# gafniguy/4D-Facial-Avatars

Hardware: AMD Instinct MI355X
Metric: rays/sec at 512x512, 64 coarse + 128 fine samples (higher is better)
Workload: dtype f32; 1 GPU; configs[1]: paper-model eval forward, 512x512 frame, 64+128 samples, chunksize 65536, perturb on, expression+latent conditioned, background prior; frames sharded over GPUs

## Files before the change

4d-facial-avatars_amd/csrc/nf_mlp_gated_stats.hip:

```cpp
#include "nf_mlp_live_kernel.h"

extern "C" int nf_paper_mlp_fwd_gated_stats(const float* packed, const float* bound, const float* cond, const float* ro, const float* rd,
                                            const float* rd_view, const float* z, int64_t n_rays, int n_samples, float* raw, float* scratch,
                                            size_t scratch_floats, int max_workgroups, int64_t* stats, size_t stats_rows, nf_stream_t stream) {
    static_assert(sizeof(long long) == sizeof(int64_t), "a statistics row is five int64");
    if (max_workgroups < 0 || !stats || ((uintptr_t)stats & 7) || stats_rows < (size_t)nf_live_grid_cap(max_workgroups) * NF_MLP_WAVES) return NF_EINVAL;
    const hipError_t e = hipMemsetAsync(stats, 0, stats_rows * NF_GATE_STAT_COLS * sizeof(int64_t), nf_s(stream));
    if (e != hipSuccess) return (int)e;
    return nf_live_launch<true, true>(packed, cond, ro, rd, rd_view, z, n_rays, n_samples, raw, scratch, scratch_floats, max_workgroups,
                                      reinterpret_cast<long long*>(stats), stream, bound);
}
```

4d-facial-avatars_amd/csrc/nf_mlp_live_kernel.h:

```cpp
#pragma once
#include <mutex>
#include "nf_mlp_paper_net.h"

#define NF_LIVE_ROWS 64
#ifndef NF_LIVE_PF
#define NF_LIVE_PF 8
#endif
#define NF_LIVE_DIR_B (NF_LIVE_ROWS * 1024)
#define NF_LIVE_META_B (NF_LIVE_DIR_B + NF_LIVE_ROWS * 64)
#define NF_LIVE_WAVE_B (NF_LIVE_META_B + NF_LIVE_ROWS * 16)
#define NF_LIVE_OOB NF_LIVE_WAVE_B
#define NF_LIVE_SC1 16

static_assert(NF_LIVE_ROWS == 64 && NF_MLP_NT == 2, "row numbers wrap with & 63; a pass's liveness is one 32-bit mask");
static_assert(NF_LIVE_PF >= 0 && NF_LIVE_PF <= 16, "prefetched rows live in registers beside fc_alpha's weights");

__device__ __forceinline__ __amdgpu_buffer_rsrc_t nf_live_ring(char* ring_v) {
    const uint64_t a = (uint64_t)ring_v;
    const uint64_t s = (uint64_t)(uint32_t)__builtin_amdgcn_readfirstlane((int)(uint32_t)a) |
                       ((uint64_t)(uint32_t)__builtin_amdgcn_readfirstlane((int)(a >> 32)) << 32);
    return __builtin_amdgcn_make_buffer_rsrc(reinterpret_cast<char*>(s), (short)0, NF_LIVE_WAVE_B, 0x00020000);
}
__device__ __forceinline__ void nf_live_store(__amdgpu_buffer_rsrc_t ring, int off_b, f32x4 v) {
    __builtin_amdgcn_raw_buffer_store_b128(__builtin_bit_cast(nf_u32x4, v), ring, off_b, 0, 0);
// ... 55 lines not shown
        const __amdgpu_buffer_rsrc_t ring = nf_live_ring(ring_v);
        const int tail = __builtin_amdgcn_readfirstlane(tail_v), cnt = __builtin_amdgcn_readfirstlane(head_v) - tail;
#pragma unroll
        for (int i = 0; i < NF_LIVE_PF; ++i)
            pf[i] = nf_live_load(ring, i < cnt ? ((tail + i) & (NF_LIVE_ROWS - 1)) * 1024 + lane * 16 : NF_LIVE_OOB);
        nf_load_bias<16>(st.bias, Ci, Net::B_FEAT, lane);
        nf_load_w16<16>(st.wa, Wi, Net::OFF_FEAT / 4, lane);
        __builtin_amdgcn_sched_barrier(0);
    }
};

#define NF_LIVE_STAT_UNITS 0
#define NF_LIVE_STAT_RUNS 1
#define NF_LIVE_STAT_FLUSH 2
#define NF_LIVE_STAT_CLOCK 3
#define NF_LIVE_STAT_COLS 4
#define NF_GATE_STAT_PROVEN 4
#define NF_GATE_STAT_COLS 5

template <bool STATS, int COLS = NF_LIVE_STAT_COLS>
__device__ __forceinline__ void nf_live_stat(long long* stats, int col, long long add, bool set = false) {
    if constexpr (STATS) {
        if ((threadIdx.x & 63) == 0) {
            long long* at = stats + ((size_t)blockIdx.x * NF_MLP_WAVES + (threadIdx.x >> 6)) * COLS + col;
            *at = set ? add : *at + add;
        }
    }
}

template <int NT, bool STATS, bool GATE = false>
__global__ void __launch_bounds__(64 * NF_MLP_WAVES, 1)
k_paper_mlp_fwd_live(const float* __restrict__ packed, const float* __restrict__ cond_, const float* __restrict__ ro,
                     const float* __restrict__ rd, const float* __restrict__ rd_view, const float* __restrict__ z,
                     int64_t n_points, int S, float* __restrict__ raw, float* __restrict__ scratch, unsigned* __restrict__ counter,
                     long long* __restrict__ stats, const float* __restrict__ bound) {
    using Net = NfPaperNet;
    constexpr int COLS = GATE ? NF_GATE_STAT_COLS : NF_LIVE_STAT_COLS;
    __shared__ __attribute__((aligned(16))) f32x4 lds[NF_MLP_WAVES * 16 * NT * 64];
    const int lane = threadIdx.x & 63, wave = threadIdx.x >> 6;
    f32x4* act4 = lds + wave * (16 * NT * 64);
    typedef __attribute__((address_space(1))) f32x4 nf_gf32x4;
    nf_gf32x4* raw_v = (nf_gf32x4*)raw;
    asm volatile("" : "+v"(raw_v));
// ... 22 lines not shown
        const bool more = __builtin_amdgcn_readfirstlane(more_v) != 0;
        unsigned next_v = 0;
        if (more && lane == 0) next_v = __hip_atomic_fetch_add(ctr_v, 1u, __ATOMIC_RELAXED, __HIP_MEMORY_SCOPE_AGENT);
        if (more) nf_live_stat<STATS, COLS>(stats, NF_LIVE_STAT_UNITS, 1);
        int opaque0 = 0;
        asm volatile("" : "+s"(opaque0));
        const NfW Wi = nf_w_image(packed + opaque0, Net::PACKED), Ci = nf_w_image(cond_ + opaque0, Net::COND_FLOATS);
        NfStream<NT> st;
        f32x4 wd[16], pf[NF_LIVE_PF > 0 ? NF_LIVE_PF : 1];
        f32x4 dirf[NT][1];
        float sigma_own[NT];
        float tag_own[NT] = {};
        bool proven[NT] = {};
        int live_v = 0, run_v = 0;
        if (more) {
            f32x4 pe[NT][4];
            nf_net_inputs<NT>(pe, dirf, p0, n_points, S, lane, ro, rd, rdv_v, z_v);
            f32x4 acc[NT][16];
            if constexpr (GATE) {
                nf_paper_net_body<Net, NT, 1, true, NfGatePre, true>(acc, sigma_own, pe, dirf, Wi, Ci, act4, lane,
                                                                     NfGatePre{st, pf, ring_v, head_v, tail_v, bound_v});
#pragma unroll
                for (int t = 0; t < NT; ++t) {
                    const float s = acc[t][8].x, u = acc[t][8].y;
                    sigma_own[t] = nf_add(s, nf_mul(u, 0x1p-13f));
                    proven[t] = sigma_own[t] < -0x1p-100f && s > -INFINITY && u < INFINITY;
                }
            } else {
                nf_paper_net_body<Net, NT, 1, true>(acc, sigma_own, pe, dirf, Wi, Ci, act4, lane, NfLivePre{st, wd, pf, ring_v, head_v, tail_v});
            }
            int lane_o = lane;
            asm volatile("" : "+v"(lane_o));
            const int g = lane_o >> 4, c = lane_o & 15;
            unsigned live = 0;
            int S_o = S;
            asm volatile("" : "+v"(S_o));
            const int64_t p0_o = (int64_t)(uint32_t)__builtin_amdgcn_readfirstlane((int)(uint32_t)p0_v) |
                                 ((int64_t)__builtin_amdgcn_readfirstlane((int)(p0_v >> 32)) << 32);
#pragma unroll
            for (int t = 0; t < NT; ++t) {
                const int64_t p = p0_o + 16 * t + c;
                const bool is_live = g == 0 && p < n_points && ((GATE ? !proven[t] : !(sigma_own[t] <= 0.0f)) || (p + 1) % S_o == 0);
                if constexpr (GATE) tag_own[t] = __int_as_float((p + 1) % S_o == 0 ? 1 : 0);
                live |= ((unsigned)__builtin_amdgcn_ballot_w64(is_live) & 0xffffu) << (16 * t);
            }
            const int head = __builtin_amdgcn_readfirstlane(head_v), cnt = head - __builtin_amdgcn_readfirstlane(tail_v);
            const int n_live = __builtin_popcount(live);
            live_v = (int)live;
            if constexpr (GATE) {
                const int64_t left = n_points - p0_o;
                nf_live_stat<STATS, COLS>(stats, NF_GATE_STAT_PROVEN, (left < 16 * NT ? (int)left : 16 * NT) - n_live);
            }
            if (cnt + n_live >= 16 * NT) {
                run_v = 1;
            } else {
                const __amdgpu_buffer_rsrc_t ring = nf_live_ring(ring_v);
                unsigned mm = live;
#pragma unroll 1
// ... 14 lines not shown
                for (int t = 0; t < NT; ++t) {
                    const int bit = 16 * t + c;
                    if ((live >> bit) & 1u) {
                        const int row = (head + __builtin_popcount(live & ((1u << bit) - 1u))) & (NF_LIVE_ROWS - 1);
                        nf_live_store(ring, NF_LIVE_DIR_B + row * 64 + g * 16, dirf[t][0]);
                        if (g == 0) {
                            const int64_t p = p0_o + bit;
                            nf_live_store(ring, NF_LIVE_META_B + row * 16,
                                          (f32x4){__int_as_float((int)(uint32_t)p), __int_as_float((int)(p >> 32)), GATE ? tag_own[t] : sigma_own[t], 0.0f});
                        }
                    }
                }
                head_v = head + n_live;
                asm volatile("" : "+v"(head_v));
            }
        } else {
            if constexpr (GATE) {
                NfGatePre pre{st, pf, ring_v, head_v, tail_v, bound_v};
                pre.wait();
                pre.loads(Wi, Ci, lane);
            } else {
                NfLivePre pre{st, wd, pf, ring_v, head_v, tail_v};
                pre.wait();
                pre.loads(Wi, Ci, lane);
            }
#pragma unroll
            for (int t = 0; t < NT; ++t) {
                dirf[t][0] = (f32x4){0.0f, 0.0f, 0.0f, 0.0f};
                sigma_own[t] = 0.0f;
            }
            run_v = __builtin_amdgcn_readfirstlane(head_v) != __builtin_amdgcn_readfirstlane(tail_v) ? 2 : 0;
        }
        asm volatile("" : "+v"(live_v), "+v"(run_v));
        const int run = __builtin_amdgcn_readfirstlane(run_v);
        if (run != 0) {
            nf_live_stat<STATS, COLS>(stats, NF_LIVE_STAT_RUNS, 1);
            if (run == 2) nf_live_stat<STATS, COLS>(stats, NF_LIVE_STAT_FLUSH, __builtin_amdgcn_readfirstlane(head_v) - __builtin_amdgcn_readfirstlane(tail_v));
            int lane_o = lane;
            asm volatile("" : "+v"(lane_o));
            const int g = lane_o >> 4, c = lane_o & 15;
            const __amdgpu_buffer_rsrc_t ring = nf_live_ring(ring_v);
            const int tail = __builtin_amdgcn_readfirstlane(tail_v), cnt = __builtin_amdgcn_readfirstlane(head_v) - tail;
            const unsigned own = run == 1 ? (unsigned)__builtin_amdgcn_readfirstlane(live_v) : 0u;
            const unsigned fill = run == 1 ? ~own : (1u << cnt) - 1u;
            const int n_fill = __builtin_popcount(fill);
            f32x4 meta[NT];
            bool valid[NT];
#pragma unroll
            for (int t = 0; t < NT; ++t) {
                const int bit = 16 * t + c;
                const bool f = (fill >> bit) & 1u;
                const int row = (tail + __builtin_popcount(fill & ((1u << bit) - 1u))) & (NF_LIVE_ROWS - 1);
// ... 17 lines not shown
                f32x4 v[4];
                int h[4];
#pragma unroll
                for (int u = 0; u < 4; ++u) {
                    const bool ok = i + u < n_fill;
                    h[u] = ok ? nf_live_pop(hh) : -1;
                    v[u] = nf_live_load(ring, ok ? ((tail + i + u) & (NF_LIVE_ROWS - 1)) * 1024 + lane_o * 16 : NF_LIVE_OOB);
                }
#pragma unroll
                for (int u = 0; u < 4; ++u)
                    if (h[u] >= 0) act4[nf_live_slab(h[u], lane_o)] = v[u];
            }
            constexpr int NDIR = 1;
            constexpr unsigned D0 = Net::OFF_D0 / 4;
            nf_read_b<NT>(st.b0, act4, lane, 0);
            f32x4 acc[NT][16], bj[NT];
            float sigma_raw[NT];
            if constexpr (GATE) {
                nf_seg_lds<NT, 16, true, true>(acc, st, Wi, Net::OFF_FEAT / 4, 16, act4, lane);
                nf_pending_b<NT, true>(bj, st);
                nf_tail<NT, 16, 16, 9, 1>(acc, st.wb, bj, st, Wi, D0, Ci, Net::B_D0, act4, lane);
                NF_NET_COLOUR();
            } else {
                NF_NET_COLOUR_D0(8, 9, wd);
                NF_NET_COLOUR_REST();
            }
            int lane_s = lane;
            asm volatile("" : "+v"(lane_s));
            if ((lane_s >> 4) == 0) {
#pragma unroll
                for (int t = 0; t < NT; ++t) {
                    if (valid[t]) {
                        const int64_t p = (int64_t)(uint32_t)__float_as_int(meta[t].x) | ((int64_t)__float_as_int(meta[t].y) << 32);
                        if constexpr (GATE) {
                            const bool keep = !(sigma_raw[t] <= 0.0f) || __float_as_int(meta[t].z) != 0;
                            if (p >= 0 && p < n_points)
                                raw_v[p] = (f32x4){keep ? acc[t][0].x : 0.0f, keep ? acc[t][0].y : 0.0f, keep ? acc[t][0].z : 0.0f, sigma_raw[t]};
                        } else {
                            if (p >= 0 && p < n_points) raw_v[p] = (f32x4){acc[t][0].x, acc[t][0].y, acc[t][0].z, meta[t].z};
                        }
                    }
                }
            }
            tail_v = tail + n_fill;
            asm volatile("" : "+v"(tail_v));
        }
        asm volatile("" : "+v"(more_v));
        if (__builtin_amdgcn_readfirstlane(more_v) == 0) break;
        {
            int lane_s = lane;
            asm volatile("" : "+v"(lane_s));
            const int g = lane_s >> 4, c = lane_s & 15;
            asm volatile("" : "+v"(live_v));
#pragma unroll
            for (int t = 0; t < NT; ++t) {
                const int64_t p = p0_v + 16 * t + c;
                if (g == 0 && p < n_points && !(((unsigned)live_v >> (16 * t + c)) & 1u)) raw_v[p] = (f32x4){0.0f, 0.0f, 0.0f, sigma_own[t]};
            }
        }
        asm volatile("" : "+v"(next_v));
        unit_v = next_v;
    }
    nf_live_stat<STATS, COLS>(stats, NF_LIVE_STAT_CLOCK, (long long)wall_clock64(), true);
}

static inline int64_t nf_live_grid_cap(int max_workgroups) {
    const int64_t cu = nf_cu_count();
    return max_workgroups > 0 && max_workgroups < cu ? max_workgroups : cu;
}

#define NF_LIVE_SLOTS 256
#define NF_LIVE_SLOT_B 128

// ... 23 lines not shown
    int i = 0;
    while (i < p.used && p.owner[i] != key) ++i;
    if (i == p.used) {
        if (p.used == NF_LIVE_SLOTS) {
            if (hipDeviceSynchronize() != hipSuccess) return nullptr;
            p.used = i = 0;
        }
        p.owner[p.used++] = key;
    }
    return reinterpret_cast<unsigned*>(p.base + (size_t)i * NF_LIVE_SLOT_B);
}

template <bool STATS, bool GATE = false>
static inline int nf_live_launch(const float* packed, const float* cond, const float* ro, const float* rd, const float* rd_view, const float* z,
                                 int64_t n_rays, int n_samples, float* raw, float* scratch, size_t scratch_floats, int max_workgroups,
                                 long long* stats, nf_stream_t stream, const float* bound = nullptr) {
    static_assert(NF_MLP_WAVES * 16 * NF_MLP_NT == 128, "nf_mlp_fwd_launch sizes the grid for 128 points per workgroup");
    if (max_workgroups < 0 || !scratch || ((uintptr_t)scratch & 15) ||
        scratch_floats < (size_t)nf_live_grid_cap(max_workgroups) * NF_MLP_WAVES * (NF_LIVE_WAVE_B / 4) ||
        (GATE && (!bound || ((uintptr_t)bound & 15))))
        return NF_EINVAL;
    const float* rdv = rd_view ? rd_view : rd;
    int rc = 0;
    const int launched = nf_mlp_fwd_launch(NF_FWD_INFER, packed, cond, ro, rd, z, raw, nullptr, n_rays, n_samples, [&](int64_t n_points, unsigned grid) {
        if ((n_points + 31) / 32 > ((int64_t)1 << 31)) {
            rc = NF_EINVAL;
            return;
        }
        unsigned* counter = nf_live_counter(nf_s(stream));
        if (!counter) {
            rc = (int)hipErrorOutOfMemory;
            return;
        }
        const hipError_t e = hipMemsetAsync(counter, 0, sizeof(unsigned), nf_s(stream));
        if (e != hipSuccess) {
            rc = (int)e;
            return;
// ... 8 lines not shown
```

4d-facial-avatars_amd/csrc/nf_mlp_live_stats.hip:

```cpp
#include "nf_mlp_live_kernel.h"

extern "C" int nf_paper_mlp_fwd_live_stats(const float* packed, const float* cond, const float* ro, const float* rd, const float* rd_view,
                                           const float* z, int64_t n_rays, int n_samples, float* raw, float* scratch, size_t scratch_floats,
                                           int max_workgroups, int64_t* stats, size_t stats_rows, nf_stream_t stream) {
    static_assert(sizeof(long long) == sizeof(int64_t), "a statistics row is four int64");
    if (max_workgroups < 0 || !stats || ((uintptr_t)stats & 7) || stats_rows < (size_t)nf_live_grid_cap(max_workgroups) * NF_MLP_WAVES) return NF_EINVAL;
    const hipError_t e = hipMemsetAsync(stats, 0, stats_rows * NF_LIVE_STAT_COLS * sizeof(int64_t), nf_s(stream));
    if (e != hipSuccess) return (int)e;
    return nf_live_launch<true>(packed, cond, ro, rd, rd_view, z, n_rays, n_samples, raw, scratch, scratch_floats, max_workgroups,
                                reinterpret_cast<long long*>(stats), stream);
}
```

4d-facial-avatars_amd/csrc/nf_mlp_paper_net.h:

```cpp
#pragma once
#include "nf_mlp_net_common.h"
#include "nf_mlp_smaller_layout.h"
#include "nf_pack.h"

#define NF_NET_COMMON(F)                                                                                                              \
    F(FRAG) F(NCOND) F(OFF_L0) F(OFF_L1) F(OFF_L2) F(OFF_L3) F(OFF_L4) F(OFF_FEAT) F(OFF_D0) F(OFF_D0E) F(OFF_D1) F(OFF_D2) F(OFF_RGB) \
    F(OFF_WC0) F(OFF_WC3) F(OFF_WCD) F(OFF_BIAS) F(B_L0) F(B_L1) F(B_L2) F(B_L3) F(B_L4) F(B_FEAT) F(B_D0) F(B_D1) F(B_D2) F(B_RGB)     \
    F(B_CVEC) F(B_DVEC) F(COND_FLOATS) F(S_PE) F(S_H0) F(S_H1) F(S_H2) F(S_H3) F(S_H4) F(S_FEAT) F(S_D0) F(S_D1) F(S_D2) F(S_DIRF)     \
    F(S_MASK) F(SAVED_PER_POINT) F(Z_L0) F(Z_L1) F(Z_L2) F(Z_L3) F(Z_L4) F(Z_FEAT) F(Z_D0) F(Z_D1) F(Z_D2) F(DZ_PER_POINT)             \
    F(OFFT_RGB) F(OFFT_D2) F(OFFT_D1) F(OFFT_D0) F(OFFT_FEAT) F(OFFT_L4) F(OFFT_L3) F(OFFT_L2) F(OFFT_L1)                              \
    F(G_L0) F(G_L1) F(G_L2) F(G_L3A) F(G_L3B) F(G_L4) F(G_FEAT) F(G_D0A) F(G_D0B) F(G_D1) F(G_D2) F(G_RGB) F(G_ALPHA)                  \
    F(CS_L0) F(CS_D0) F(CS_RGB) F(SLAB_FLOATS) F(GRAD_PARAM_FLOATS) F(GRAD_FLOATS)

struct NfPaperNet {
#define NF_NET_COPY(X) static constexpr int X = nfl::X;
    NF_NET_COMMON(NF_NET_COPY)
    NF_NET_COPY(OFF_L5) NF_NET_COPY(B_L5) NF_NET_COPY(S_H5) NF_NET_COPY(Z_L5) NF_NET_COPY(OFFT_L5) NF_NET_COPY(G_L5)
#undef NF_NET_COPY
    static constexpr bool HAS_L5 = true, D0_EXPR = false;
    static constexpr int PACKED = nfl::PACKED_FLOATS, PACKED_T = nfl::PACKED_T_FLOATS, NPARAMS = NF_PAPER_NUM_PARAMS;
    static constexpr int N_RELU = (nfl::SAVED_PER_POINT - nfl::S_MASK) / 8;
    static constexpr int D0_COLS = 280;
    static constexpr int MODEL = 0;
};
// ... 181 lines not shown

struct NfNoPre {
    __device__ __forceinline__ void wait() const {}
    __device__ __forceinline__ void loads(const NfW&, const NfW&, int) const {}
};
#define NF_BOUND_BIAS 4096
#define NF_BOUND_FLOATS (NF_BOUND_BIAS + 16)
template <int NT, bool RELU_IN, class Pre>
__device__ __forceinline__ void nf_net_lone_tile(f32x4 (&acc)[NT][16], const NfStream<NT>& st, f32x4 (&bj)[NT], const NfW& W, unsigned first4,
                                                 unsigned stride4, const NfW& Wi, const NfW& Ci, const f32x4* act4, int lane, Pre& pre) {
    f32x4 w8[16];
    w8[0] = st.wa[0];
    pre.wait();
#pragma unroll
    for (int ch = 1; ch < 16; ++ch) w8[ch] = nf_load_w1(W, first4 + stride4 * ch, lane);
    pre.loads(Wi, Ci, lane);
#pragma unroll
    for (int ch = 0; ch < 16; ++ch) {
        if (ch == 0) {
#pragma unroll
            for (int t = 0; t < NT; ++t) bj[t] = RELU_IN ? nf_relu_i(st.b0[t]) : st.b0[t];
        } else {
            nf_read_b<NT>(bj, act4, lane, ch);
            if (RELU_IN) {
#pragma unroll
                for (int t = 0; t < NT; ++t) bj[t] = nf_relu_i(bj[t]);
            }
        }
#pragma unroll
        for (int r = 0; r < 4; ++r)
#pragma unroll
// ... 236 lines not shown
```

4d-facial-avatars_amd/nerf/_hip.py:

```python
from __future__ import annotations

import ctypes as C
import os
import threading

import torch

_LIB_PATH = os.environ.get("NERFACE_HIP_LIB") or os.path.join(os.path.dirname(os.path.dirname(os.path.abspath(__file__))), "lib",
                                                             "libnerface_hip.so")
_lib = None
_lock = threading.Lock()

NF_PAPER_NUM_PARAMS = 26

_P, _I, _L, _F, _Z = C.c_void_p, C.c_int, C.c_int64, C.c_float, C.c_size_t
_PROTOTYPES = {
    "nf_abi_version": (C.c_int, []),
    "nf_error_string": (C.c_char_p, [_I]),
    "nf_build_info": (C.c_char_p, []),
    "nf_ray_bundle": (C.c_int, [_I, _I, _F, _F, _F, _F, _P, _I, _P, _P, _P]),
    "nf_weighted_choice_workspace_bytes": (_Z, []),
    "nf_weighted_choice": (C.c_int, [_P, _P, _L, _I, _P, _P, _Z, _P]),
    "nf_ray_batch": (C.c_int, [_I, _I, _F, _F, _F, _F, _P, _I, _P, _I, _L, _P, _I, _P, _P, _P, _P, _P, _P, _P]),
    "nf_sample_coarse": (C.c_int, [_L, _I, _F, _F, _P, _P, _P, _P]),
# ... 151 lines not shown
    "forward_encoded": (C.c_int, [_P, _P, _P, _P, _L, _P, _P, _P]),
}
for _prefix in ("nf_bshape", "nf_cbshape"):
    _PROTOTYPES.update({f"{_prefix}_{_name}": _sig for _name, _sig in _FAMILY_ENTRY_POINTS.items()})
_SIGMA_SIG = (C.c_int, [_P, _P, _P, _P, _P, _P, _L, _I, _P, _P])
SIGMA_ENTRY_POINTS = tuple(f"{_prefix}_mlp_sigma{_suffix}" for _prefix in ("nf_paper", "nf_lcode", "nf_bshape", "nf_cbshape")
                           for _suffix in ("", "_bf16", "_f16", "_f16x2")) + ("nf_smaller_mlp_sigma",)
_PROTOTYPES.update({_name: _SIGMA_SIG for _name in SIGMA_ENTRY_POINTS})
_PROTOTYPES["nf_volume_weights_fwd"] = (C.c_int, [_P, _P, _P, _P, _L, _I, _P, _P, _P, _P])
_PROTOTYPES["nf_paper_mlp_fwd_live_scratch_floats"] = (_Z, [_I])
_PROTOTYPES["nf_paper_mlp_fwd_live"] = (C.c_int, [_P, _P, _P, _P, _P, _P, _L, _I, _P, _P, _Z, _I, _P])
_PROTOTYPES["nf_paper_mlp_fwd_live_stats"] = (C.c_int, [_P, _P, _P, _P, _P, _P, _L, _I, _P, _P, _Z, _I, _P, _Z, _P])
_PROTOTYPES["nf_paper_sigma_bound_floats"] = (_Z, [])
_PROTOTYPES["nf_paper_sigma_bound"] = (C.c_int, [_P, _P, _P])
_PROTOTYPES["nf_paper_mlp_fwd_gated"] = (C.c_int, [_P, _P, _P, _P, _P, _P, _P, _L, _I, _P, _P, _Z, _I, _P])
_PROTOTYPES["nf_paper_mlp_fwd_gated_stats"] = (C.c_int, [_P, _P, _P, _P, _P, _P, _P, _L, _I, _P, _P, _Z, _I, _P, _Z, _P])
_PROTOTYPES["nf_isosurface_workspace_bytes"] = (_Z, [_I, _I, _I])
_PROTOTYPES["nf_isosurface_count"] = (C.c_int, [_P, _I, _I, _I, _F, _P, _Z, _P, _P])
_PROTOTYPES["nf_isosurface_emit"] = (C.c_int, [_P, _I, _I, _I, _F, _P, _P, _P, _Z, _P, _L, _P, _L, _P, _P])
_PROTOTYPES["nf_isosurface_table"] = (C.c_int, [_P])
_PROTOTYPES["nf_sparse_grid_workspace_bytes"] = (_Z, [_I, _I, _I, _I])
_PROTOTYPES["nf_sparse_grid_lattice"] = (C.c_int, [_I, _I, _I, _I, _P, _P, _P, _P, _L, _P])
_PROTOTYPES["nf_sparse_grid_classify"] = (C.c_int, [_P, _I, _I, _I, _I, _F, _F, _I, _P, _Z, _P])
_PROTOTYPES["nf_sparse_grid_mark"] = (C.c_int, [_I, _I, _I, _I, _P, _Z, _P, _P])
_PROTOTYPES["nf_sparse_grid_emit"] = (C.c_int, [_P, _I, _I, _I, _I, _P, _P, _P, _Z, _P, _P, _L, _P])
_PROTOTYPES["nf_sparse_grid_scatter"] = (C.c_int, [_P, _P, _L, _P, _I, _I, _I, _P])
for _prefix in ("nf_lcode", "nf_bshape", "nf_cbshape"):
    _PROTOTYPES[f"{_prefix}_mlp_bwd_stage_ms"] = (C.c_int, [_P, _P, _I, _P, _P, _P, _L, _I, _P, _Z, _P, _P, _P])
_OPTIONAL = set()
ABI_VERSION = 5

# ... 64 lines not shown
```

4d-facial-avatars_amd/nerf/ops.py:

```python
from __future__ import annotations

import ctypes as C
import os
import weakref
from typing import NamedTuple, Optional, Sequence

import numpy as np
import torch

from . import _hip as H

PAPER_KEYS = (
    [f"layers_xyz.{i}.{p}" for i in range(6) for p in ("weight", "bias")]
    + [f"{n}.{p}" for n in ("fc_feat", "fc_alpha") for p in ("weight", "bias")]
    + [f"layers_dir.{i}.{p}" for i in range(4) for p in ("weight", "bias")]
    + [f"fc_rgb.{p}" for p in ("weight", "bias")]
)
LCODE_KEYS = [f"{n}.{p}" for n in ("layer1", "layers_xyz.0", "layers_xyz.1", "layers_xyz.2", "layers_dir.0", "fc_alpha", "fc_rgb", "fc_feat")
              for p in ("weight", "bias")]
SMALLER_KEYS = [f"{n}.{p}" for n in ([f"layers_xyz.{i}" for i in range(5)] + ["fc_feat", "fc_alpha"] + [f"layers_dir.{i}" for i in range(3)]
                                     + ["fc_rgb"]) for p in ("weight", "bias")]
BSHAPE_KEYS = list(LCODE_KEYS)
CBSHAPE_KEYS = [f"layers_expr.{i}.{p}" for i in range(3) for p in ("weight", "bias")] + LCODE_KEYS

# ... 348 lines not shown
        raise NotImplementedError(f"the {fam.prefix} model family has no live-colour kernel")
    dev = H.require_device(packed, cond, ro, rd, z, rd_view)
    n_rays, n_samples = z.shape
    raw = torch.empty((n_rays, n_samples, 4), dtype=torch.float32, device=dev)
    with torch.cuda.device(dev):
        key = (dev, H.stream_ptr(dev), int(max_workgroups))
        scratch = _LIVE_SCRATCH.get(key)
        if scratch is None:
            scratch = _LIVE_SCRATCH[key] = torch.empty(fam.fn("mlp_fwd_live_scratch_floats")(int(max_workgroups)), dtype=torch.float32, device=dev)
        fam.call("mlp_fwd_live", H.ptr(packed), H.ptr(cond), H.ptr(ro), H.ptr(rd), H.ptr(rd_view), H.ptr(z), n_rays, n_samples, H.ptr(raw),
                 H.ptr(scratch), scratch.numel(), int(max_workgroups), H.stream_ptr(dev))
    _live_launches[0] += 1
    return raw


LIVE_STAT_COLUMNS = ("units", "colour_runs", "flush_rows", "exit_clock")


def mlp_fwd_live_stats(fam: MLPFamily, packed, cond, ro, rd, z, rd_view=None, max_workgroups: int = 0):
    if fam.prefix not in LIVE_FAMILIES:
        raise NotImplementedError(f"the {fam.prefix} model family has no live-colour kernel")
    dev = H.require_device(packed, cond, ro, rd, z, rd_view)
    n_rays, n_samples = z.shape
    raw = torch.empty((n_rays, n_samples, 4), dtype=torch.float32, device=dev)
    with torch.cuda.device(dev):
        scratch = torch.empty(fam.fn("mlp_fwd_live_scratch_floats")(int(max_workgroups)), dtype=torch.float32, device=dev)
        waves = scratch.numel() * 4 // (LIVE_RING_ROWS * LIVE_ROW_BYTES)
        stats = torch.empty((waves, len(LIVE_STAT_COLUMNS)), dtype=torch.int64, device=dev)
        fam.call("mlp_fwd_live_stats", H.ptr(packed), H.ptr(cond), H.ptr(ro), H.ptr(rd), H.ptr(rd_view), H.ptr(z), n_rays, n_samples,
                 H.ptr(raw), H.ptr(scratch), scratch.numel(), int(max_workgroups), stats.data_ptr(), waves, H.stream_ptr(dev))
    return raw, stats


GATED_PASSES_DEFAULT = ("coarse",)
_gated_passes = (set(GATED_PASSES_DEFAULT) if os.environ.get("NERFACE_SIGMA_GATE") is None
                 else {p for p in os.environ["NERFACE_SIGMA_GATE"].split(",") if p in ("coarse", "fine")})
_gated_launches = [0]
GATED_STAT_COLUMNS = LIVE_STAT_COLUMNS + ("proven_rows",)


def set_sigma_gate(on, passes=("coarse", "fine")) -> None:
    global _gated_passes
    _gated_passes = set(GATED_PASSES_DEFAULT) if on is None else (set(passes) if on else set())


def sigma_gate_applies(fam: MLPFamily, which: str) -> bool:
    return which in _gated_passes and live_colour_kernel(fam)


def live_mode(fam: MLPFamily, which: str):
    if sigma_gate_applies(fam, which):
        return "gated"
    return live_colour_applies(fam, which)
# ... 33 lines not shown
        _gated_call("mlp_fwd_gated", fam, packed, bound, cond, ro, rd, z, rd_view, max_workgroups, scratch, raw, H.stream_ptr(dev))
    _gated_launches[0] += 1
    return raw


def mlp_fwd_gated_stats(fam: MLPFamily, packed, bound, cond, ro, rd, z, rd_view=None, max_workgroups: int = 0):
    if fam.prefix not in LIVE_FAMILIES:
        raise NotImplementedError(f"the {fam.prefix} model family has no gated kernel")
    dev = H.require_device(packed, bound, cond, ro, rd, z, rd_view)
    n_rays, n_samples = z.shape
    raw = torch.empty((n_rays, n_samples, 4), dtype=torch.float32, device=dev)
    with torch.cuda.device(dev):
        scratch = torch.empty(fam.fn("mlp_fwd_live_scratch_floats")(int(max_workgroups)), dtype=torch.float32, device=dev)
        waves = scratch.numel() * 4 // (LIVE_RING_ROWS * LIVE_ROW_BYTES)
        stats = torch.empty((waves, len(GATED_STAT_COLUMNS)), dtype=torch.int64, device=dev)
        _gated_call("mlp_fwd_gated_stats", fam, packed, bound, cond, ro, rd, z, rd_view, max_workgroups, scratch, raw, stats.data_ptr(), waves,
                    H.stream_ptr(dev))
    return raw, stats


_SIGMA_ENTRY = {"f32": "mlp_sigma", "bf16x3": "mlp_sigma_bf16", "f16x3": "mlp_sigma_f16", "f16x2": "mlp_sigma_f16x2"}


def mlp_sigma(fam: MLPFamily, precision: str, image, cond, ro, rd, z) -> torch.Tensor:
    dev = H.require_device(image if precision == "f32" else None, cond, ro, rd, z)
    n_rays, n_samples = z.shape
    sigma = torch.empty((n_rays, n_samples), dtype=torch.float32, device=dev)
    with torch.cuda.device(dev):
        fam.call(_SIGMA_ENTRY[precision], H.ptr(image), H.ptr(cond), H.ptr(ro), H.ptr(rd), 0, H.ptr(z), n_rays, n_samples, H.ptr(sigma),
                 H.stream_ptr(dev))
    return sigma
# ... 667 lines not shown
```

include/nerface_hip.h:

```cpp
#ifndef NERFACE_HIP_H
#define NERFACE_HIP_H

#include <stddef.h>
#include <stdint.h>

#ifdef __cplusplus
extern "C" {
#endif

typedef void* nf_stream_t;

#define NF_EINVAL (-22)

int         nf_abi_version(void);
const char* nf_error_string(int code);
const char* nf_build_info(void);

int nf_ray_bundle(int height, int width, float fx, float fy, float cx_w, float cy_h,
                  const float* c2w, int c2w_row_stride, float* ro, float* rd, nf_stream_t stream);

int nf_ray_batch(int height, int width, float fx, float fy, float cx_w, float cy_h, const float* c2w, int c2w_row_stride,
                 const int64_t* sel, int sel_is_flat, int64_t n, const float* image, int channels, const float* bg, float* ro,
                 float* rd, float* target, float* bg_out, int* bad_flag, nf_stream_t stream);

// ... 356 lines not shown
                              const float* z, int64_t n_rays, int n_samples, float* sigma, nf_stream_t stream);
NF_DECLARE_MLP_SIGMA(nf_paper) NF_DECLARE_MLP_SIGMA_SPLIT(nf_paper)
NF_DECLARE_MLP_SIGMA(nf_lcode) NF_DECLARE_MLP_SIGMA_SPLIT(nf_lcode)
NF_DECLARE_MLP_SIGMA(nf_bshape) NF_DECLARE_MLP_SIGMA_SPLIT(nf_bshape)
NF_DECLARE_MLP_SIGMA(nf_cbshape) NF_DECLARE_MLP_SIGMA_SPLIT(nf_cbshape)
NF_DECLARE_MLP_SIGMA(nf_smaller)
#undef NF_DECLARE_MLP_SIGMA
#undef NF_DECLARE_MLP_SIGMA_SPLIT
int nf_volume_weights_fwd(const float* sigma, const float* z, const float* rd, const float* noise, int64_t n_rays, int n_samples,
                          float* disp, float* acc, float* weights, nf_stream_t stream);

size_t nf_paper_mlp_fwd_live_scratch_floats(int max_workgroups);
int nf_paper_mlp_fwd_live(const float* packed, const float* cond, const float* ro, const float* rd, const float* rd_view,
                          const float* z, int64_t n_rays, int n_samples, float* raw, float* scratch, size_t scratch_floats,
                          int max_workgroups, nf_stream_t stream);
int nf_paper_mlp_fwd_live_stats(const float* packed, const float* cond, const float* ro, const float* rd, const float* rd_view,
                                const float* z, int64_t n_rays, int n_samples, float* raw, float* scratch, size_t scratch_floats,
                                int max_workgroups, int64_t* stats, size_t stats_rows, nf_stream_t stream);

size_t nf_paper_sigma_bound_floats(void);
int nf_paper_sigma_bound(const float* packed, float* bound, nf_stream_t stream);
int nf_paper_mlp_fwd_gated(const float* packed, const float* bound, const float* cond, const float* ro, const float* rd,
                           const float* rd_view, const float* z, int64_t n_rays, int n_samples, float* raw, float* scratch,
                           size_t scratch_floats, int max_workgroups, nf_stream_t stream);
int nf_paper_mlp_fwd_gated_stats(const float* packed, const float* bound, const float* cond, const float* ro, const float* rd,
                                 const float* rd_view, const float* z, int64_t n_rays, int n_samples, float* raw, float* scratch,
                                 size_t scratch_floats, int max_workgroups, int64_t* stats, size_t stats_rows, nf_stream_t stream);

size_t nf_isosurface_workspace_bytes(int nx, int ny, int nz);
int nf_isosurface_count(const float* grid, int nx, int ny, int nz, float level, void* workspace, size_t workspace_bytes,
                        int64_t* counts_dev, nf_stream_t stream);
int nf_isosurface_emit(const float* grid, int nx, int ny, int nz, float level, const float* lo, const float* hi, void* workspace,
                       size_t workspace_bytes, float* verts, int64_t n_verts, int* faces, int64_t n_faces, float* normals,
                       nf_stream_t stream);
// ... 30 lines not shown
```

Before: 612,200 rays/s.

## Gate fine pass by sigma bound, pipeline relu-input layer, add phase clocks

Turns on the sigma-bound gate for the fine pass as well as the coarse pass by default, so rows proven empty skip the colour head in both passes. Restructures the relu-input trunk layer so each chunk's LDS activation read and ReLU overlap with the MFMAs of the previous chunk. Also adds per-phase clock instrumentation and atomic stat updates for profiling builds, tagged through the low bit of the stats pointer. The gate adds bound work in the fine pass and skips only where the bound holds, and the new schedule barriers may raise register pressure.

```diff
diff --git a/4d-facial-avatars_amd/csrc/nf_mlp_gated_stats.hip b/4d-facial-avatars_amd/csrc/nf_mlp_gated_stats.hip
--- a/4d-facial-avatars_amd/csrc/nf_mlp_gated_stats.hip
+++ b/4d-facial-avatars_amd/csrc/nf_mlp_gated_stats.hip
@@ -1,12 +1,27 @@
 #include "nf_mlp_live_kernel.h"
+
+static int nf_gated_stats_launch(bool clocks, const float* packed, const float* bound, const float* cond, const float* ro, const float* rd,
+                                 const float* rd_view, const float* z, int64_t n_rays, int n_samples, float* raw, float* scratch,
+                                 size_t scratch_floats, int max_workgroups, int64_t* stats, size_t stats_rows, nf_stream_t stream) {
+    static_assert(sizeof(long long) == sizeof(int64_t), "a statistics row is int64s");
+    if (max_workgroups < 0 || !stats || ((uintptr_t)stats & 7) || stats_rows < (size_t)nf_live_grid_cap(max_workgroups) * NF_MLP_WAVES) return NF_EINVAL;
+    const size_t cols = NF_GATE_STAT_COLS + (clocks ? NF_LIVE_PHASES : 0);
+    const hipError_t e = hipMemsetAsync(stats, 0, stats_rows * cols * sizeof(int64_t), nf_s(stream));
+    if (e != hipSuccess) return (int)e;
+    return nf_live_launch<true, true>(packed, cond, ro, rd, rd_view, z, n_rays, n_samples, raw, scratch, scratch_floats, max_workgroups,
+                                      reinterpret_cast<long long*>(stats), stream, bound, clocks);
+}
 
 extern "C" int nf_paper_mlp_fwd_gated_stats(const float* packed, const float* bound, const float* cond, const float* ro, const float* rd,
                                             const float* rd_view, const float* z, int64_t n_rays, int n_samples, float* raw, float* scratch,
                                             size_t scratch_floats, int max_workgroups, int64_t* stats, size_t stats_rows, nf_stream_t stream) {
-    static_assert(sizeof(long long) == sizeof(int64_t), "a statistics row is five int64");
-    if (max_workgroups < 0 || !stats || ((uintptr_t)stats & 7) || stats_rows < (size_t)nf_live_grid_cap(max_workgroups) * NF_MLP_WAVES) return NF_EINVAL;
-    const hipError_t e = hipMemsetAsync(stats, 0, stats_rows * NF_GATE_STAT_COLS * sizeof(int64_t), nf_s(stream));
-    if (e != hipSuccess) return (int)e;
-    return nf_live_launch<true, true>(packed, cond, ro, rd, rd_view, z, n_rays, n_samples, raw, scratch, scratch_floats, max_workgroups,
-                                      reinterpret_cast<long long*>(stats), stream, bound);
+    return nf_gated_stats_launch(false, packed, bound, cond, ro, rd, rd_view, z, n_rays, n_samples, raw, scratch, scratch_floats, max_workgroups,
+                                 stats, stats_rows, stream);
 }
+
+extern "C" int nf_paper_mlp_fwd_gated_phases(const float* packed, const float* bound, const float* cond, const float* ro, const float* rd,
+                                             const float* rd_view, const float* z, int64_t n_rays, int n_samples, float* raw, float* scratch,
+                                             size_t scratch_floats, int max_workgroups, int64_t* stats, size_t stats_rows, nf_stream_t stream) {
+    return nf_gated_stats_launch(true, packed, bound, cond, ro, rd, rd_view, z, n_rays, n_samples, raw, scratch, scratch_floats, max_workgroups,
+                                 stats, stats_rows, stream);
+}
diff --git a/4d-facial-avatars_amd/csrc/nf_mlp_live_kernel.h b/4d-facial-avatars_amd/csrc/nf_mlp_live_kernel.h
--- a/4d-facial-avatars_amd/csrc/nf_mlp_live_kernel.h
+++ b/4d-facial-avatars_amd/csrc/nf_mlp_live_kernel.h
@@ -93,19 +93,54 @@
 #define NF_LIVE_STAT_RUNS 1
 #define NF_LIVE_STAT_FLUSH 2
 #define NF_LIVE_STAT_CLOCK 3
+#define NF_GATE_STAT_PROVEN 4
+#define NF_LIVE_PH_TRUNK 0
+#define NF_LIVE_PH_TILE 1
+#define NF_LIVE_PH_APPEND 2
+#define NF_LIVE_PH_ENTRY 3
+#define NF_LIVE_PH_RUN 4
+#define NF_LIVE_PH_DEAD 5
+#define NF_LIVE_PHASES 6
 #define NF_LIVE_STAT_COLS 4
-#define NF_GATE_STAT_PROVEN 4
 #define NF_GATE_STAT_COLS 5
 
 template <bool STATS, int COLS = NF_LIVE_STAT_COLS>
 __device__ __forceinline__ void nf_live_stat(long long* stats, int col, long long add, bool set = false) {
     if constexpr (STATS) {
+        const int cols = COLS + (((uintptr_t)stats & 1) ? NF_LIVE_PHASES : 0);
+        stats = reinterpret_cast<long long*>((uintptr_t)stats & ~(uintptr_t)7);
         if ((threadIdx.x & 63) == 0) {
-            long long* at = stats + ((size_t)blockIdx.x * NF_MLP_WAVES + (threadIdx.x >> 6)) * COLS + col;
-            *at = set ? add : *at + add;
-        }
-    }
-}
+            long long* at = stats + ((size_t)blockIdx.x * NF_MLP_WAVES + (threadIdx.x >> 6)) * cols + col;
+            if (set) *at = add;
+            else (void)__hip_atomic_fetch_add(at, add, __ATOMIC_RELAXED, __HIP_MEMORY_SCOPE_AGENT);
+        }
+    }
+}
+
+template <bool STATS, int COLS>
+__device__ __forceinline__ void nf_live_mark(long long* stats, int end, int start) {
+    if constexpr (STATS) {
+        if ((uintptr_t)stats & 1) {
+            __builtin_amdgcn_sched_barrier(0);
+            const long long t = (long long)__builtin_amdgcn_s_memtime();
+            if ((threadIdx.x & 63) == 0) {
+                long long* row = reinterpret_cast<long long*>((uintptr_t)stats & ~(uintptr_t)7) +
+                                 ((size_t)blockIdx.x * NF_MLP_WAVES + (threadIdx.x >> 6)) * (COLS + NF_LIVE_PHASES) + COLS;
+                if (end >= 0) (void)__hip_atomic_fetch_add(row + end, t, __ATOMIC_RELAXED, __HIP_MEMORY_SCOPE_AGENT);
+                if (start >= 0) (void)__hip_atomic_fetch_add(row + start, -t, __ATOMIC_RELAXED, __HIP_MEMORY_SCOPE_AGENT);
+            }
+            __builtin_amdgcn_sched_barrier(0);
+        }
+    }
+}
+template <class Pre, int COLS>
+struct NfMarkedPre : Pre {
+    long long* stats;
+    __device__ __forceinline__ void wait() const {
+        nf_live_mark<true, COLS>(stats, NF_LIVE_PH_TRUNK, NF_LIVE_PH_TILE);
+        Pre::wait();
+    }
+};
 
 template <int NT, bool STATS, bool GATE = false>
 __global__ void __launch_bounds__(64 * NF_MLP_WAVES, 1)
@@ -158,21 +193,30 @@
         bool proven[NT] = {};
         int live_v = 0, run_v = 0;
         if (more) {
+            nf_live_mark<STATS, COLS>(stats, -1, NF_LIVE_PH_TRUNK);
             f32x4 pe[NT][4];
             nf_net_inputs<NT>(pe, dirf, p0, n_points, S, lane, ro, rd, rdv_v, z_v);
             f32x4 acc[NT][16];
             if constexpr (GATE) {
-                nf_paper_net_body<Net, NT, 1, true, NfGatePre, true>(acc, sigma_own, pe, dirf, Wi, Ci, act4, lane,
-                                                                     NfGatePre{st, pf, ring_v, head_v, tail_v, bound_v});
+                if constexpr (STATS)
+                    nf_paper_net_body<Net, NT, 1, true, NfMarkedPre<NfGatePre, COLS>, true>(
+                        acc, sigma_own, pe, dirf, Wi, Ci, act4, lane, NfMarkedPre<NfGatePre, COLS>{{st, pf, ring_v, head_v, tail_v, bound_v}, stats});
+                else
+                    nf_paper_net_body<Net, NT, 1, true, NfGatePre, true>(acc, sigma_own, pe, dirf, Wi, Ci, act4, lane,
+                                                                         NfGatePre{st, pf, ring_v, head_v, tail_v, bound_v});
 #pragma unroll
                 for (int t = 0; t < NT; ++t) {
                     const float s = acc[t][8].x, u = acc[t][8].y;
                     sigma_own[t] = nf_add(s, nf_mul(u, 0x1p-13f));
                     proven[t] = sigma_own[t] < -0x1p-100f && s > -INFINITY && u < INFINITY;
                 }
+            } else if constexpr (STATS) {
+                nf_paper_net_body<Net, NT, 1, true>(acc, sigma_own, pe, dirf, Wi, Ci, act4, lane,
+                                                    NfMarkedPre<NfLivePre, COLS>{{st, wd, pf, ring_v, head_v, tail_v}, stats});
             } else {
                 nf_paper_net_body<Net, NT, 1, true>(acc, sigma_own, pe, dirf, Wi, Ci, act4, lane, NfLivePre{st, wd, pf, ring_v, head_v, tail_v});
             }
+            nf_live_mark<STATS, COLS>(stats, NF_LIVE_PH_TILE, NF_LIVE_PH_APPEND);
             int lane_o = lane;
             asm volatile("" : "+v"(lane_o));
             const int g = lane_o >> 4, c = lane_o & 15;
@@ -184,8 +228,14 @@
 #pragma unroll
             for (int t = 0; t < NT; ++t) {
                 const int64_t p = p0_o + 16 * t + c;
-                const bool is_live = g == 0 && p < n_points && ((GATE ? !proven[t] : !(sigma_own[t] <= 0.0f)) || (p + 1) % S_o == 0);
-                if constexpr (GATE) tag_own[t] = __int_as_float((p + 1) % S_o == 0 ? 1 : 0);
+                bool is_live;
+                if constexpr (GATE) {
+                    const bool last = (p + 1) % S_o == 0;
+                    is_live = g == 0 && p < n_points && (!proven[t] || last);
+                    tag_own[t] = __int_as_float(last ? 1 : 0);
+                } else {
+                    is_live = g == 0 && p < n_points && (!(sigma_own[t] <= 0.0f) || (p + 1) % S_o == 0);
+                }
                 live |= ((unsigned)__builtin_amdgcn_ballot_w64(is_live) & 0xffffu) << (16 * t);
             }
             const int head = __builtin_amdgcn_readfirstlane(head_v), cnt = head - __builtin_amdgcn_readfirstlane(tail_v);
@@ -230,6 +280,7 @@
                 head_v = head + n_live;
                 asm volatile("" : "+v"(head_v));
             }
+            nf_live_mark<STATS, COLS>(stats, NF_LIVE_PH_APPEND, -1);
         } else {
             if constexpr (GATE) {
                 NfGatePre pre{st, pf, ring_v, head_v, tail_v, bound_v};
@@ -252,6 +303,7 @@
         if (run != 0) {
             nf_live_stat<STATS, COLS>(stats, NF_LIVE_STAT_RUNS, 1);
             if (run == 2) nf_live_stat<STATS, COLS>(stats, NF_LIVE_STAT_FLUSH, __builtin_amdgcn_readfirstlane(head_v) - __builtin_amdgcn_readfirstlane(tail_v));
+            nf_live_mark<STATS, COLS>(stats, -1, NF_LIVE_PH_ENTRY);
             int lane_o = lane;
             asm volatile("" : "+v"(lane_o));
             const int g = lane_o >> 4, c = lane_o & 15;
@@ -299,6 +351,7 @@
             constexpr int NDIR = 1;
             constexpr unsigned D0 = Net::OFF_D0 / 4;
             nf_read_b<NT>(st.b0, act4, lane, 0);
+            nf_live_mark<STATS, COLS>(stats, NF_LIVE_PH_ENTRY, NF_LIVE_PH_RUN);
             f32x4 acc[NT][16], bj[NT];
             float sigma_raw[NT];
             if constexpr (GATE) {
@@ -329,10 +382,12 @@
             }
             tail_v = tail + n_fill;
             asm volatile("" : "+v"(tail_v));
+            nf_live_mark<STATS, COLS>(stats, NF_LIVE_PH_RUN, -1);
         }
         asm volatile("" : "+v"(more_v));
         if (__builtin_amdgcn_readfirstlane(more_v) == 0) break;
         {
+            nf_live_mark<STATS, COLS>(stats, -1, NF_LIVE_PH_DEAD);
             int lane_s = lane;
             asm volatile("" : "+v"(lane_s));
             const int g = lane_s >> 4, c = lane_s & 15;
@@ -342,6 +397,7 @@
                 const int64_t p = p0_v + 16 * t + c;
                 if (g == 0 && p < n_points && !(((unsigned)live_v >> (16 * t + c)) & 1u)) raw_v[p] = (f32x4){0.0f, 0.0f, 0.0f, sigma_own[t]};
             }
+            nf_live_mark<STATS, COLS>(stats, NF_LIVE_PH_DEAD, -1);
         }
         asm volatile("" : "+v"(next_v));
         unit_v = next_v;
@@ -395,13 +451,14 @@
 template <bool STATS, bool GATE = false>
 static inline int nf_live_launch(const float* packed, const float* cond, const float* ro, const float* rd, const float* rd_view, const float* z,
                                  int64_t n_rays, int n_samples, float* raw, float* scratch, size_t scratch_floats, int max_workgroups,
-                                 long long* stats, nf_stream_t stream, const float* bound = nullptr) {
+                                 long long* stats, nf_stream_t stream, const float* bound = nullptr, bool clocks = false) {
     static_assert(NF_MLP_WAVES * 16 * NF_MLP_NT == 128, "nf_mlp_fwd_launch sizes the grid for 128 points per workgroup");
     if (max_workgroups < 0 || !scratch || ((uintptr_t)scratch & 15) ||
         scratch_floats < (size_t)nf_live_grid_cap(max_workgroups) * NF_MLP_WAVES * (NF_LIVE_WAVE_B / 4) ||
         (GATE && (!bound || ((uintptr_t)bound & 15))))
         return NF_EINVAL;
     const float* rdv = rd_view ? rd_view : rd;
+    if (STATS && clocks) stats = reinterpret_cast<long long*>((uintptr_t)stats | 1);
     int rc = 0;
     const int launched = nf_mlp_fwd_launch(NF_FWD_INFER, packed, cond, ro, rd, z, raw, nullptr, n_rays, n_samples, [&](int64_t n_points, unsigned grid) {
         if ((n_points + 31) / 32 > ((int64_t)1 << 31)) {
diff --git a/4d-facial-avatars_amd/csrc/nf_mlp_live_stats.hip b/4d-facial-avatars_amd/csrc/nf_mlp_live_stats.hip
--- a/4d-facial-avatars_amd/csrc/nf_mlp_live_stats.hip
+++ b/4d-facial-avatars_amd/csrc/nf_mlp_live_stats.hip
@@ -1,12 +1,27 @@
 #include "nf_mlp_live_kernel.h"
+
+static int nf_live_stats_launch(bool clocks, const float* packed, const float* cond, const float* ro, const float* rd, const float* rd_view,
+                                const float* z, int64_t n_rays, int n_samples, float* raw, float* scratch, size_t scratch_floats,
+                                int max_workgroups, int64_t* stats, size_t stats_rows, nf_stream_t stream) {
+    static_assert(sizeof(long long) == sizeof(int64_t), "a statistics row is int64s");
+    if (max_workgroups < 0 || !stats || ((uintptr_t)stats & 7) || stats_rows < (size_t)nf_live_grid_cap(max_workgroups) * NF_MLP_WAVES) return NF_EINVAL;
+    const size_t cols = NF_LIVE_STAT_COLS + (clocks ? NF_LIVE_PHASES : 0);
+    const hipError_t e = hipMemsetAsync(stats, 0, stats_rows * cols * sizeof(int64_t), nf_s(stream));
+    if (e != hipSuccess) return (int)e;
+    return nf_live_launch<true>(packed, cond, ro, rd, rd_view, z, n_rays, n_samples, raw, scratch, scratch_floats, max_workgroups,
+                                reinterpret_cast<long long*>(stats), stream, nullptr, clocks);
+}
 
 extern "C" int nf_paper_mlp_fwd_live_stats(const float* packed, const float* cond, const float* ro, const float* rd, const float* rd_view,
                                            const float* z, int64_t n_rays, int n_samples, float* raw, float* scratch, size_t scratch_floats,
                                            int max_workgroups, int64_t* stats, size_t stats_rows, nf_stream_t stream) {
-    static_assert(sizeof(long long) == sizeof(int64_t), "a statistics row is four int64");
-    if (max_workgroups < 0 || !stats || ((uintptr_t)stats & 7) || stats_rows < (size_t)nf_live_grid_cap(max_workgroups) * NF_MLP_WAVES) return NF_EINVAL;
-    const hipError_t e = hipMemsetAsync(stats, 0, stats_rows * NF_LIVE_STAT_COLS * sizeof(int64_t), nf_s(stream));
-    if (e != hipSuccess) return (int)e;
-    return nf_live_launch<true>(packed, cond, ro, rd, rd_view, z, n_rays, n_samples, raw, scratch, scratch_floats, max_workgroups,
-                                reinterpret_cast<long long*>(stats), stream);
+    return nf_live_stats_launch(false, packed, cond, ro, rd, rd_view, z, n_rays, n_samples, raw, scratch, scratch_floats, max_workgroups, stats,
+                                stats_rows, stream);
 }
+
+extern "C" int nf_paper_mlp_fwd_live_phases(const float* packed, const float* cond, const float* ro, const float* rd, const float* rd_view,
+                                            const float* z, int64_t n_rays, int n_samples, float* raw, float* scratch, size_t scratch_floats,
+                                            int max_workgroups, int64_t* stats, size_t stats_rows, nf_stream_t stream) {
+    return nf_live_stats_launch(true, packed, cond, ro, rd, rd_view, z, n_rays, n_samples, raw, scratch, scratch_floats, max_workgroups, stats,
+                                stats_rows, stream);
+}
diff --git a/4d-facial-avatars_amd/csrc/nf_mlp_paper_net.h b/4d-facial-avatars_amd/csrc/nf_mlp_paper_net.h
--- a/4d-facial-avatars_amd/csrc/nf_mlp_paper_net.h
+++ b/4d-facial-avatars_amd/csrc/nf_mlp_paper_net.h
@@ -219,7 +219,43 @@
     pre.wait();
 #pragma unroll
     for (int ch = 1; ch < 16; ++ch) w8[ch] = nf_load_w1(W, first4 + stride4 * ch, lane);
+    if constexpr (RELU_IN) __builtin_amdgcn_sched_barrier(0);
     pre.loads(Wi, Ci, lane);
+    if constexpr (RELU_IN) {
+        f32x4 cur[NT], nxt[NT];
+#pragma unroll
+        for (int t = 0; t < NT; ++t) cur[t] = nf_relu_i(st.b0[t]);
+#pragma unroll
+        for (int ch = 0; ch < 16; ++ch) {
+            if (ch + 1 < 16) nf_read_b<NT>(nxt, act4, lane, ch + 1);
+            __builtin_amdgcn_sched_barrier(0);
+#pragma unroll
+            for (int r = 0; r < 2; ++r)
+#pragma unroll
+                for (int t = 0; t < NT; ++t)
+                    acc[t][8] = __builtin_amdgcn_mfma_f32_16x16x4f32(w8[ch][r], cur[t][r], (ch == 0 && r == 0) ? st.bias[0] : acc[t][8], 0, 0, 0);
+#pragma unroll
+            for (int r = 2; r < 4; ++r)
+#pragma unroll
+                for (int t = 0; t < NT; ++t) {
+                    __builtin_amdgcn_sched_barrier(0);
+                    if (ch + 1 < 16) {
+                        const int e = 2 * (r - 2);
+#pragma unroll
+                        for (int q = e; q < e + 2; ++q) {
+                            const int xi = __float_as_int(nxt[t][q]);
+                            nxt[t][q] = __int_as_float(xi > 0 ? xi : 0);
+                        }
+                    }
+                    __builtin_amdgcn_sched_barrier(0);
+                    acc[t][8] = __builtin_amdgcn_mfma_f32_16x16x4f32(w8[ch][r], cur[t][r], acc[t][8], 0, 0, 0);
+                }
+            __builtin_amdgcn_sched_barrier(0);
+#pragma unroll
+            for (int t = 0; t < NT; ++t) cur[t] = nxt[t];
+        }
+        return;
+    }
 #pragma unroll
     for (int ch = 0; ch < 16; ++ch) {
         if (ch == 0) {
diff --git a/4d-facial-avatars_amd/nerf/_hip.py b/4d-facial-avatars_amd/nerf/_hip.py
--- a/4d-facial-avatars_amd/nerf/_hip.py
+++ b/4d-facial-avatars_amd/nerf/_hip.py
@@ -189,7 +189,9 @@
 _PROTOTYPES["nf_paper_sigma_bound_floats"] = (_Z, [])
 _PROTOTYPES["nf_paper_sigma_bound"] = (C.c_int, [_P, _P, _P])
 _PROTOTYPES["nf_paper_mlp_fwd_gated"] = (C.c_int, [_P, _P, _P, _P, _P, _P, _P, _L, _I, _P, _P, _Z, _I, _P])
+_PROTOTYPES["nf_paper_mlp_fwd_live_phases"] = _PROTOTYPES["nf_paper_mlp_fwd_live_stats"]
 _PROTOTYPES["nf_paper_mlp_fwd_gated_stats"] = (C.c_int, [_P, _P, _P, _P, _P, _P, _P, _L, _I, _P, _P, _Z, _I, _P, _Z, _P])
+_PROTOTYPES["nf_paper_mlp_fwd_gated_phases"] = _PROTOTYPES["nf_paper_mlp_fwd_gated_stats"]
 _PROTOTYPES["nf_isosurface_workspace_bytes"] = (_Z, [_I, _I, _I])
 _PROTOTYPES["nf_isosurface_count"] = (C.c_int, [_P, _I, _I, _I, _F, _P, _Z, _P, _P])
 _PROTOTYPES["nf_isosurface_emit"] = (C.c_int, [_P, _I, _I, _I, _F, _P, _P, _P, _Z, _P, _L, _P, _L, _P, _P])
diff --git a/4d-facial-avatars_amd/nerf/ops.py b/4d-facial-avatars_amd/nerf/ops.py
--- a/4d-facial-avatars_amd/nerf/ops.py
+++ b/4d-facial-avatars_amd/nerf/ops.py
@@ -386,7 +386,8 @@
     return raw
 
 
-LIVE_STAT_COLUMNS = ("units", "colour_runs", "flush_rows", "exit_clock")
+LIVE_PHASE_COLUMNS = ("clk_trunk", "clk_lone_tile", "clk_append", "clk_run_entry", "clk_run", "clk_dead_stores")
+LIVE_STAT_COLUMNS = ("units", "colour_runs", "flush_rows", "exit_clock") + LIVE_PHASE_COLUMNS
 
 
 def mlp_fwd_live_stats(fam: MLPFamily, packed, cond, ro, rd, z, rd_view=None, max_workgroups: int = 0):
@@ -399,16 +400,16 @@
         scratch = torch.empty(fam.fn("mlp_fwd_live_scratch_floats")(int(max_workgroups)), dtype=torch.float32, device=dev)
         waves = scratch.numel() * 4 // (LIVE_RING_ROWS * LIVE_ROW_BYTES)
         stats = torch.empty((waves, len(LIVE_STAT_COLUMNS)), dtype=torch.int64, device=dev)
-        fam.call("mlp_fwd_live_stats", H.ptr(packed), H.ptr(cond), H.ptr(ro), H.ptr(rd), H.ptr(rd_view), H.ptr(z), n_rays, n_samples,
+        fam.call("mlp_fwd_live_phases", H.ptr(packed), H.ptr(cond), H.ptr(ro), H.ptr(rd), H.ptr(rd_view), H.ptr(z), n_rays, n_samples,
                  H.ptr(raw), H.ptr(scratch), scratch.numel(), int(max_workgroups), stats.data_ptr(), waves, H.stream_ptr(dev))
     return raw, stats
 
 
-GATED_PASSES_DEFAULT = ("coarse",)
+GATED_PASSES_DEFAULT = ("coarse", "fine")
 _gated_passes = (set(GATED_PASSES_DEFAULT) if os.environ.get("NERFACE_SIGMA_GATE") is None
                  else {p for p in os.environ["NERFACE_SIGMA_GATE"].split(",") if p in ("coarse", "fine")})
 _gated_launches = [0]
-GATED_STAT_COLUMNS = LIVE_STAT_COLUMNS + ("proven_rows",)
+GATED_STAT_COLUMNS = LIVE_STAT_COLUMNS[:4] + ("proven_rows",) + LIVE_PHASE_COLUMNS
 
 
 def set_sigma_gate(on, passes=("coarse", "fine")) -> None:
@@ -472,7 +473,7 @@
         scratch = torch.empty(fam.fn("mlp_fwd_live_scratch_floats")(int(max_workgroups)), dtype=torch.float32, device=dev)
         waves = scratch.numel() * 4 // (LIVE_RING_ROWS * LIVE_ROW_BYTES)
         stats = torch.empty((waves, len(GATED_STAT_COLUMNS)), dtype=torch.int64, device=dev)
-        _gated_call("mlp_fwd_gated_stats", fam, packed, bound, cond, ro, rd, z, rd_view, max_workgroups, scratch, raw, stats.data_ptr(), waves,
+        _gated_call("mlp_fwd_gated_phases", fam, packed, bound, cond, ro, rd, z, rd_view, max_workgroups, scratch, raw, stats.data_ptr(), waves,
                     H.stream_ptr(dev))
     return raw, stats
 
diff --git a/include/nerface_hip.h b/include/nerface_hip.h
--- a/include/nerface_hip.h
+++ b/include/nerface_hip.h
@@ -394,10 +394,16 @@
 int nf_paper_mlp_fwd_live(const float* packed, const float* cond, const float* ro, const float* rd, const float* rd_view,
                           const float* z, int64_t n_rays, int n_samples, float* raw, float* scratch, size_t scratch_floats,
                           int max_workgroups, nf_stream_t stream);
+int nf_paper_mlp_fwd_live_phases(const float* packed, const float* cond, const float* ro, const float* rd, const float* rd_view,
+                                 const float* z, int64_t n_rays, int n_samples, float* raw, float* scratch, size_t scratch_floats,
+                                 int max_workgroups, int64_t* stats, size_t stats_rows, nf_stream_t stream);
 int nf_paper_mlp_fwd_live_stats(const float* packed, const float* cond, const float* ro, const float* rd, const float* rd_view,
                                 const float* z, int64_t n_rays, int n_samples, float* raw, float* scratch, size_t scratch_floats,
                                 int max_workgroups, int64_t* stats, size_t stats_rows, nf_stream_t stream);
 
+int nf_paper_mlp_fwd_gated_phases(const float* packed, const float* bound, const float* cond, const float* ro, const float* rd,
+                                  const float* rd_view, const float* z, int64_t n_rays, int n_samples, float* raw, float* scratch,
+                                  size_t scratch_floats, int max_workgroups, int64_t* stats, size_t stats_rows, nf_stream_t stream);
 size_t nf_paper_sigma_bound_floats(void);
 int nf_paper_sigma_bound(const float* packed, float* bound, nf_stream_t stream);
 int nf_paper_mlp_fwd_gated(const float* packed, const float* bound, const float* cond, const float* ro, const float* rd,
```

New measurement: 621,900 rays/s, median of 6. 1.02x the previous value.
